# BICLab/Spike2Former

Measured on AMD Instinct MI355X. Metric: fwd+bwd images/sec, 512x512 T=4 ADE20K-150, higher is better.
Workload: dtype f32 (fp32-equivalent: bf16 hi+mid+lo split operands on bf16 MFMA, fp32 accumulate; spike maps stored as bf16, exact); 1 GPU; C2: 512x512 T=4 K=150 Meta-SpikeFormer [64, 128, 256, 360] + MaskFormer head, per-GPU batch 2; global_batch=2, parallelism=dp1, weights=random-init (name-seeded)

## Files before the change

include/s2f.h:

```cpp
#ifndef S2F_H
#define S2F_H

#include <stdint.h>

#ifdef __cplusplus
extern "C" {
#endif

#define S2F_OK 0
#define S2F_EINVAL (-1)
#define S2F_EALIGN (-2)
#define S2F_ELAUNCH (-3)

#define S2F_ABI_VERSION 53
#define S2F_STAT_SLOTS 256

int s2f_version(void);
const char* s2f_last_error(void);

void* s2f_event_create(void);
void s2f_event_destroy(void* event);
int s2f_time_next_call(void* start_event, void* stop_event);
int s2f_event_elapsed_us(void* start_event, void* stop_event, double* microseconds);

int64_t s2f_lif_mask_words(int64_t n);

int s2f_lif_fwd(const float* x, const float* v_in, void* y, float* v_out, uint64_t* mask, uint8_t* count_u8,
                uint64_t* stats, int64_t n, float vth, int D, int y_bf16, void* stream);

int s2f_lif_bwd(const float* gy, const float* gv_out, const uint64_t* mask, float* gx, int64_t n, float vth, int D,
                void* stream);
int s2f_lif_bwd_ports(const float* gy, const float* gy2, const float* gv_out, const uint64_t* mask, const float* skip, float* gx,
                      int64_t n, float vth, int D, void* stream);

int s2f_lif_leaky_fwd(const float* x, const float* v_in, void* y, float* v_out, uint64_t* mask, uint64_t* stats, int64_t n, float vth,
                      int D, float tau, int decay_input, int y_bf16, void* stream);
int s2f_lif_leaky_bwd(const float* gy, const float* gv_out, const uint64_t* mask, float* gx, float* gv_in, int64_t n, float vth, int D,
                      float tau, int decay_input, void* stream);

int s2f_sum2_lif_fwd(const float* x, const float* e, const float* pos, void* y_key, void* y_value, uint64_t* mask_key,
                     uint64_t* mask_value, int64_t TB, int64_t B, int64_t C, int64_t L, float vth, int D, int y_bf16,
                     void* stream);
int s2f_sum2_lif_bwd(const float* g_key, const float* g_value, const uint64_t* mask_key, const uint64_t* mask_value,
                     float* gx, int64_t n, int D, void* stream);
int s2f_sum2_lif_bwd_ex(const float* g_key, const float* g_value, const uint64_t* mask_key, const uint64_t* mask_value, float* gx,
                        float* gx_key, int64_t n, int D, void* stream);
int s2f_sum2_lif_bwd_ports(const float* g_key, const float* g_key2, const float* g_value, const float* g_value2,
                           const uint64_t* mask_key, const uint64_t* mask_value, const float* skip, float* gx, float* gx_key, int64_t n,
                           int D, void* stream);

int s2f_scale_affine_fwd(const float* gamma, const float* beta, const float* s, float* w, float* b, int C, void* stream);
int s2f_scale_affine_bwd(const float* gw, const float* gb, const float* gamma, const float* beta, const float* s,
                         float* dgamma, float* dbeta, float* ds, int C, void* stream);

int s2f_lif_seq_fwd(const float* x_seq, const float* v0, float* y_seq, float* vT, uint64_t* mask, uint64_t* stats,
                    int T, int64_t n, float vth, int D, void* stream);
int s2f_lif_seq_bwd(const float* gy_seq, const float* gvT, const uint64_t* mask, float* gx_seq, float* gv0, int T,
                    int64_t n, float vth, int D, void* stream);

int s2f_bn_single_pass(int64_t N, int64_t C, int64_t L);
int64_t s2f_bn_mask_words(int64_t N, int64_t C, int64_t L);
int s2f_bn_stats(const float* z, const float* conv_bias, double* sums_zeroed, int64_t N, int64_t C, int64_t L,
                 void* stream);
int s2f_bn_act_fwd(const float* z, const float* conv_bias, const double* sums, float* stat_out, float* running_mean,
                   float* running_var, int64_t* num_batches_tracked, const float* gamma, const float* beta,
                   const float* residual, float* u_out, const float* v_in, void* y, float* v_out, uint64_t* mask,
                   uint64_t* stats, int64_t N, int64_t C, int64_t L, float momentum, float eps, int training, float vth,
                   int D, int y_bf16, void* stream);
int s2f_bn_act_bwd(const float* z, const float* conv_bias, const float* stat, const float* gamma, const float* g_u,
                   const float* g_y, const float* g_v, const uint64_t* mask, double* sums_zeroed, float* gz,
                   float* g_residual, float* dgamma, float* dbeta, int64_t N, int64_t C, int64_t L, int training,
                   float vth, int D, void* stream);
int s2f_bn_up_ok(int64_t N, int64_t C, int64_t H, int64_t W, int training, int D);
int s2f_bn_act_up_fwd(const float* z, const float* conv_bias, const double* sums, float* stat_out, float* running_mean,
                      float* running_var, int64_t* num_batches_tracked, const float* gamma, const float* beta,
                      const float* residual_lo, float* u_out, const float* v_in, void* y, float* v_out, uint64_t* mask,
                      uint64_t* stats, int64_t N, int64_t C, int64_t H, int64_t W, float momentum, float eps, int training,
                      float vth, int D, int y_bf16, void* stream);

int s2f_bn2_fused_ok(int64_t N, int64_t C, int64_t L);
int s2f_bn2_act_fwd(const float* z, const float* conv_bias, float* stat_out, float* running_mean, float* running_var,
                    int64_t* num_batches_tracked, const float* gamma, const float* beta, float momentum, float eps,
                    const float* gamma2, const float* beta2, float* running_mean2, float* running_var2,
                    int64_t* num_batches_tracked2, float momentum2, float eps2, const float* residual, float* u_out,
                    const float* v_in, void* y, float* v_out, uint64_t* mask, uint64_t* stats, int64_t N, int64_t C, int64_t L,
                    float vth, int D, int y_bf16, void* stream);
int s2f_bn2_act_bwd(const float* z, const float* conv_bias, const float* stat, const float* gamma, const float* gamma2, float eps2,
                    const float* g_u, const float* g_y, const float* g_v, const uint64_t* mask, float* gz, float* g_residual,
                    float* dgamma, float* dbeta, float* dgamma2, float* dbeta2, int64_t N, int64_t C, int64_t L, float vth, int D,
                    void* stream);

int s2f_im2col(const void* x, void* cols, int N, int C, int H, int W, int kh, int kw, int stride, int pad, int x_bf16, void* stream);
int s2f_col2im(const float* cols, float* gx, int N, int C, int H, int W, int kh, int kw, int stride, int pad, void* stream);
// ... 326 lines not shown
```

spike2former_amd/_lib.py:

```python
import ctypes
import os

import torch

_HERE = os.path.dirname(os.path.abspath(__file__))
LIB_PATH = os.environ.get("S2F_LIB") or os.path.join(_HERE, "libs2f_hip.so")

_p, _i, _i64, _f = ctypes.c_void_p, ctypes.c_int, ctypes.c_int64, ctypes.c_float

SIGNATURES = {
    "s2f_version": (_i, []),
    "s2f_last_error": (ctypes.c_char_p, []),
    "s2f_event_create": (_p, []),
    "s2f_event_destroy": (None, [_p]),
    "s2f_time_next_call": (_i, [_p, _p]),
    "s2f_event_elapsed_us": (_i, [_p, _p, ctypes.POINTER(ctypes.c_double)]),
    "s2f_lif_mask_words": (_i64, [_i64]),
    "s2f_lif_fwd": (_i, [_p, _p, _p, _p, _p, _p, _p, _i64, _f, _i, _i, _p]),
    "s2f_lif_bwd": (_i, [_p, _p, _p, _p, _i64, _f, _i, _p]),
    "s2f_lif_bwd_ports": (_i, [_p] * 6 + [_i64, _f, _i, _p]),
    "s2f_lif_leaky_fwd": (_i, [_p, _p, _p, _p, _p, _p, _i64, _f, _i, _f, _i, _i, _p]),
    "s2f_lif_leaky_bwd": (_i, [_p, _p, _p, _p, _p, _i64, _f, _i, _f, _i, _p]),
    "s2f_sum2_lif_fwd": (_i, [_p] * 7 + [_i64] * 4 + [_f, _i, _i, _p]),
    "s2f_sum2_lif_bwd": (_i, [_p] * 5 + [_i64, _i, _p]),
    "s2f_sum2_lif_bwd_ex": (_i, [_p] * 6 + [_i64, _i, _p]),
    "s2f_sum2_lif_bwd_ports": (_i, [_p] * 9 + [_i64, _i, _p]),
    "s2f_mask_loss_fwd": (_i, [_p] * 4 + [_i64, _i, _i, _f, _f, _p]),
    "s2f_mask_loss_bwd": (_i, [_p] * 5 + [_i64, _i, _i, _f, _f, _p]),
    "s2f_scale_affine_fwd": (_i, [_p] * 5 + [_i, _p]),
    "s2f_scale_affine_bwd": (_i, [_p] * 8 + [_i, _p]),
    "s2f_lif_seq_fwd": (_i, [_p, _p, _p, _p, _p, _p, _i, _i64, _f, _i, _p]),
    "s2f_lif_seq_bwd": (_i, [_p, _p, _p, _p, _p, _i, _i64, _f, _i, _p]),
    "s2f_bn_single_pass": (_i, [_i64] * 3),
    "s2f_bn_mask_words": (_i64, [_i64] * 3),
    "s2f_bn2_fused_ok": (_i, [_i64] * 3),
    "s2f_bn2_act_fwd": (_i, [_p] * 8 + [_f, _f] + [_p] * 5 + [_f, _f] + [_p] * 7 + [_i64] * 3 + [_f, _i, _i, _p]),
    "s2f_bn2_act_bwd": (_i, [_p] * 5 + [_f] + [_p] * 10 + [_i64] * 3 + [_f, _i, _p]),
    "s2f_bn_stats": (_i, [_p] * 3 + [_i64] * 3 + [_p]),
    "s2f_bn_act_fwd": (_i, [_p] * 16 + [_i64] * 3 + [_f, _f, _i, _f, _i, _i, _p]),
    "s2f_bn_act_bwd": (_i, [_p] * 13 + [_i64] * 3 + [_i, _f, _i, _p]),
    "s2f_bn_up_ok": (_i, [_i64] * 4 + [_i, _i]),
    "s2f_bn_act_up_fwd": (_i, [_p] * 16 + [_i64] * 4 + [_f, _f, _i, _f, _i, _i, _p]),
    "s2f_im2col": (_i, [_p, _p] + [_i] * 9 + [_p]),
    "s2f_col2im": (_i, [_p, _p] + [_i] * 8 + [_p]),
    "s2f_dwconv_fwd": (_i, [_p] * 4 + [_i] * 7 + [_p]),
    "s2f_dwconv_stats_slots": (_i64, [_i] * 3),
    "s2f_dwconv_fwd_stats": (_i, [_p] * 4 + [_i64] + [_i] * 5 + [_p]),
    "s2f_dwconv_bn_lif_fwd": (_i, [_p] * 7 + [_f] + [_p] * 3 + [_i] * 7 + [_f, _i, _p]),
    "s2f_dwconv_bwd_input": (_i, [_p] * 3 + [_i] * 6 + [_p]),
    "s2f_dwconv_bwd_weight": (_i, [_p] * 4 + [_i] * 8 + [_p]),
    "s2f_split_bf16x3": (_i, [_p, _p, _i, _i, _i, _i, _p]),
    "s2f_split_bf16x3_multi": (_i, [_p, _i, _i64, _p]),
    "s2f_spike_gemm_fwd": (_i, [_p] * 4 + [_i] * 7 + [_p]),
    "s2f_upsample2x_fwd": (_i, [_p, _p, _i64, _i, _i, _p]),
    "s2f_upsample2x_sigmoid_fwd": (_i, [_p, _p, _i64, _i, _i, _p]),
    "s2f_upsample2x_bwd": (_i, [_p, _p, _i64, _i, _i, _p]),
    "s2f_upsample2x_bwd_add": (_i, [_p, _p, _p, _i64, _i, _i, _p]),
    "s2f_resize_fwd": (_i, [_p, _p, _i64, _i64] + [_i] * 8 + [_p]),
    "s2f_resize_bwd_add": (_i, [_p, _p, _p, _i64] + [_i] * 5 + [_p]),
    "s2f_seg_argmax": (_i, [_p, _p, _p, _i, _i64, _i, _f, _p]),
    "s2f_seg_label": (_i, [_p, _p, _p, _i, _i64] + [_i] * 8 + [_f, _p]),
    "s2f_tta_accumulate": (_i, [_p, _p, _i, _i64] + [_i] * 9 + [_p]),
    "s2f_tta_finish": (_i, [_p, _p, _p, _i, _i64, _i, _f, _p]),
    "s2f_slide_windows": (_i, [_p, _p] + [_i] * 10 + [_p]),
    "s2f_slide_accumulate": (_i, [_p, _p] + [_i] * 10 + [_p]),
    "s2f_seg_hist": (_i, [_p, _i, _p, _i, _i64, _i64, _i, _i64, _i, _i, _i, _p, _p]),
# ... 138 lines not shown
```

spike2former_amd/csrc/bn_lif.hip:

```cpp
#include "gemm_common.h"
#include <cstring>

namespace {

constexpr int kBlock = 256;
constexpr int kWaves = kBlock / S2F_WAVE;

__device__ __forceinline__ double wave_sum_f64(double v) {
  for (int o = 32; o > 0; o >>= 1) v += __shfl_xor(v, o, 64);
  return v;
}

__device__ __forceinline__ void block_atomic_add2(double a, double b, double* dst, double pivot = 0.0, double count = 0.0) {
  __shared__ double red[2 * kWaves];
  a = wave_sum_f64(a);
  b = wave_sum_f64(b);
  const int lane = threadIdx.x & 63, w = threadIdx.x >> 6;
  if (lane == 0) {
    red[2 * w] = a;
    red[2 * w + 1] = b;
  }
  __syncthreads();
  if (threadIdx.x == 0) {
    double sa = 0, sb = 0;
// ... 1067 lines not shown
        }
      }
      if (u_out) st4(u_out + base[i], uo);
      if (LIF) {
        if (YB)
          st4_bf16(y, base[i], yo);
        else
          st4(y + base[i], yo);
        if (v_out) st4(v_out + base[i], vo);
        const uint64_t b0 = __ballot(inr[0]), b1 = __ballot(inr[1]), b2 = __ballot(inr[2]), b3 = __ballot(inr[3]);
        const int64_t tile = base[i] >> 8;
        if (mask != nullptr && lane < 4) mask[tile * 4 + lane] = lane == 0 ? b0 : lane == 1 ? b1 : lane == 2 ? b2 : b3;
      }
    }
  }
  if (LIF && stats != nullptr) {
    double a = (double)csum, bq = (double)cnz;
    block_sum2(a, bq, red, nwaves);
    if (threadIdx.x == 0) {
      unsigned long long* slot = stats + 2 * (blockIdx.x % S2F_STAT_SLOTS);
      if (a > 0) atomicAdd(&slot[0], (unsigned long long)a);
      if (bq > 0) atomicAdd(&slot[1], (unsigned long long)bq);
    }
  }
}

struct Bn2Bwd {
  const float* gamma;
  float* dgamma;
  float* dbeta;
  float eps;
};

template <bool GU, bool GY, bool GV, bool DOUBLE = false>
__global__ __launch_bounds__(kFusedBlock) void bn_fused_bwd_kernel(
    const float* __restrict__ z, const float* __restrict__ bias, const float* __restrict__ stat,
    const float* __restrict__ gamma, const float* __restrict__ g_u, const float* __restrict__ g_y,
    const float* __restrict__ g_v, const uint64_t* __restrict__ mask, float* __restrict__ gz, float* __restrict__ g_res,
    float* __restrict__ dgamma, float* __restrict__ dbeta, int N, int C, int L, double inv_count, float vth, float Df,
    unsigned short* __restrict__ gzs, Bn2Bwd bn2, const float* __restrict__ g_y2) {
  __shared__ double red[2 * kFusedWaves];
  const int c = blockIdx.x, lane = threadIdx.x & 63, w = threadIdx.x >> 6, nwaves = blockDim.x >> 6;
  const int tpr = L >> 8, tiles = N * tpr;
  const float b = bias ? bias[c] : 0.f, mean = stat[c], rstd = stat[C + c], g = gamma[c];
  Tile4 xh[kTpw], gu[kTpw];
  int tix[kTpw];
#pragma unroll
  for (int i = 0; i < kTpw; ++i) {
    const int t = w + i * nwaves;
    tix[i] = t < tiles ? t : -1;
    const int tt = t < tiles ? t : 0;
    const int n = tt / tpr, q = tt - n * tpr;
    const int64_t base = ((int64_t)n * C + c) * L + q * 256 + lane * 4;
    xh[i] = (S2F_BN_NT & 16) ? ld4_nt(z + base) : ld4(z + base);
    if (GU) gu[i] = (S2F_BN_NT & 16) ? ld4_nt(g_u + base) : ld4(g_u + base);
    Tile4 bb, cc;
    uint64_t word = 0;
    if (GY) bb = (S2F_BN_NT & 16) ? ld4_nt(g_y + base) : ld4(g_y + base);
    if (GY && g_y2) {
      const Tile4 t2 = (S2F_BN_NT & 16) ? ld4_nt(g_y2 + base) : ld4(g_y2 + base);
#pragma unroll
      for (int j = 0; j < 4; ++j) bb.a[j] += t2.a[j];
    }
    if (GV) cc = ld4(g_v + base);
    if (GY || GV) word = mask[(base >> 8) * 4 + (lane & 3)];
#pragma unroll
    for (int j = 0; j < 4; ++j) {
      bool m = false;
      if (GY || GV) {
        const uint32_t lo = __shfl((uint32_t)word, j, 64), hi = __shfl((uint32_t)(word >> 32), j, 64);
        m = ((lane < 32 ? lo >> lane : hi >> (lane - 32)) & 1u) != 0;
      }
      gu[i].a[j] = form_gu(GU, GU ? gu[i].a[j] : 0.f, GY, GY ? bb.a[j] : 0.f, GV, GV ? cc.a[j] : 0.f, m, vth, Df);
      xh[i].a[j] = ((xh[i].a[j] + b) - mean) * rstd;
    }
  }
  float ps = 0.f, pq = 0.f;
#pragma unroll
  for (int i = 0; i < kTpw; ++i) {
    if (tix[i] < 0) continue;
#pragma unroll
    for (int j = 0; j < 4; ++j) {
      ps += gu[i].a[j];
      pq += gu[i].a[j] * xh[i].a[j];
    }
  }
  double s1 = (double)ps, s2 = (double)pq;
  block_sum2(s1, s2, red, nwaves);
  float scale = g * rstd;
  float m1 = (float)(s1 * inv_count), m2 = (float)(s2 * inv_count);
  if constexpr (DOUBLE) {
    const float r_c = stat[3 * C + c], g_c = bn2.gamma[c];
    if (threadIdx.x == 0) {
      bn2.dbeta[c] = (float)s1;
      bn2.dgamma[c] = (g * r_c) * (float)s2;
      dbeta[c] = 0.f;
      dgamma[c] = (g_c * bn2.eps) * (r_c * r_c * r_c) * (float)s2;
    }
    scale = (g * rstd) * (g_c * r_c);
    m2 *= (r_c * r_c) * (g * g + bn2.eps);
  } else if (threadIdx.x == 0) {
    dbeta[c] = (float)s1;
    dgamma[c] = (float)s2;
  }
#pragma unroll
  for (int i = 0; i < kTpw; ++i) {
    if (tix[i] < 0) continue;
    const int n = tix[i] / tpr, q = tix[i] - n * tpr;
    const int64_t base = ((int64_t)n * C + c) * L + q * 256 + lane * 4;
    Tile4 o;
#pragma unroll
    for (int j = 0; j < 4; ++j) o.a[j] = scale * ((gu[i].a[j] - m1) - xh[i].a[j] * m2);
    store_gz(gz, gzs, (int64_t)N * C * L, base, o);
    if (g_res) st4(g_res + base, gu[i]);
  }
}

constexpr int kSmallIters = 8;

inline bool small_rows_ok(int64_t N, int64_t C, int64_t L) {
  return (L & 3) == 0 && (L & 255) != 0 && N * L <= 64 * 4 * kSmallIters && N * L >= 8 && C >= 32;
}

template <bool LIF, bool HAS_V, bool YB, bool GROUPED = false>
__global__ __launch_bounds__(64) void bn_small_fwd_kernel(
    const float* __restrict__ z, const float* __restrict__ bias, float* __restrict__ stat, float* __restrict__ running_mean,
    float* __restrict__ running_var, long long* __restrict__ num_batches, const float* __restrict__ gamma,
    const float* __restrict__ beta, const float* __restrict__ res, float* __restrict__ u_out, const float* __restrict__ v_in,
    float* __restrict__ y, float* __restrict__ v_out, uint64_t* __restrict__ mask, unsigned long long* __restrict__ stats,
    int N, int C, int L, double inv_count, float unbias, float momentum, float eps, float vth, float Df) {
  if constexpr (GROUPED) {
    static_assert(!HAS_V, "grouped form: neurons from rest");
    const int64_t g = blockIdx.y, map = g * N * C * L, vec = g * C;
    z += map;
    if (bias) bias += vec;
    stat += 3 * vec;
    if (running_mean) running_mean += vec, running_var += vec;
    gamma += vec, beta += vec;
    if (u_out) u_out += map;
// ... 339 lines not shown
  const float m1 = (float)(s1 * inv_count), m2 = (float)(s2 * inv_count);
#pragma unroll
  for (int i = 0; i < kMidIters; ++i) {
    if (!ok[i]) continue;
    Tile4 o;
#pragma unroll
    for (int j = 0; j < 4; ++j) o.a[j] = (g_ * rstd) * ((gu[i].a[j] - m1) - xh[i].a[j] * m2);
    st4(gz + base[i], o);
    if (g_res) st4(g_res + base[i], gu[i]);
  }
}

inline bool single_pass_ok(int64_t N, int64_t C, int64_t L) {
  if ((L & 255) != 0) return false;
  const int64_t tiles = N * (L >> 8);
  return tiles >= 4 && tiles <= kFusedWaves * kTpw && C >= 64 && N * C * L < ((int64_t)1 << 31);
}
inline int single_pass_threads(int64_t N, int64_t L) {
  const int tiles = (int)(N * (L >> 8));
  return 64 * ((tiles + kTpw - 1) / kTpw);
}

inline int pick_slices(int C, int L, int& slice) {
  int S = 1;
  while ((int64_t)C * S < 1024 && L / (S * 2) >= 2048) S *= 2;
  slice = ((L + S - 1) / S + 3) / 4 * 4;
  return S;
}

inline bool rows_ok(int64_t N, int64_t C, int64_t L, int D) {
  return (L & 3) == 0 && L >= 256 && N * C * L < ((int64_t)1 << 39) && N * C < ((int64_t)1 << 31) && D >= 1 && (D & (D - 1)) == 0;
}
inline bool rows_aligned(int64_t total, int64_t L) { return (L & 255) == 0 && (total & 255) == 0; }
inline bool up_ok(int64_t N, int64_t C, int64_t L, int64_t H, int64_t W, int training, int D) {
  return training && rows_ok(N, C, L, D) && rows_aligned(N * C * L, L) && !single_pass_ok(N, C, L) && H > 0 && W > 0 && H * W == L &&
         (H & 1) == 0 && (W & 3) == 0 && (W < 256 ? 256 % W == 0 : W % 256 == 0) && W < (1 << 24);
}
inline int pick_slices_rows(int C, int L, int& slice) {
  int S = 1;
  while ((int64_t)C * S < 2048 && L / (S * 2) >= 2048) S *= 2;
  slice = ((L + S - 1) / S + 255) / 256 * 256;
  return (L + slice - 1) / slice;
}
template <auto Kern>
int resident_blocks(size_t lds) {
  static int cus = 0, per_cu_small = 0;
  if (cus == 0) {
    int dev = 0;
    if (hipGetDevice(&dev) != hipSuccess || hipDeviceGetAttribute(&cus, hipDeviceAttributeMultiprocessorCount, dev) != hipSuccess ||
        cus < 1)
      cus = 256;
  }
  int per_cu = lds <= 16384 ? per_cu_small : 0;
  if (per_cu == 0) {
    if (hipOccupancyMaxActiveBlocksPerMultiprocessor(&per_cu, Kern, kBlock, lds <= 16384 ? 16384 : lds) != hipSuccess || per_cu < 1)
      per_cu = 4;
    if (lds <= 16384) per_cu_small = per_cu;
  }
  return cus * per_cu;
}
template <auto Kern>
int grid_rows(uint32_t ntiles, size_t lds, uint32_t& chunk, int want) {
  static const char* env = getenv("S2F_BN_ROWS_CHUNK");
  if (env != nullptr) {
    const int fwd_want = atoi(env), bwd_want = strchr(env, ',') ? atoi(strchr(env, ',') + 1) : fwd_want;
    want = want == 8 ? fwd_want : bwd_want;
// ... 32 lines not shown
    {true, true, true},
};
template <class F>
void for_fwd_variant(const float* y, const float* v_in, int y_bf16, const F& launch) {
  s2f_dispatch<kFwdVariants>(
      [&](const FwdVariant& e) {
        return y ? (e.lif && e.has_v == (v_in != nullptr) && e.yb == (y_bf16 != 0)) : !e.lif;
      },
      launch);
}

struct BwdGrads {
  bool gu, gy, gv;
};
constexpr BwdGrads kBwdGrads[] = {
    {false, false, true},
    {false, true, false},
    {false, true, true},
    {true, false, false},
    {true, false, true},
    {true, true, false},
    {true, true, true},
};
template <class F>
void for_bwd_grads(const float* g_u, const float* g_y, const float* g_v, const F& launch) {
  s2f_dispatch<kBwdGrads>(
      [&](const BwdGrads& e) { return e.gu == (g_u != nullptr) && e.gy == (g_y != nullptr) && e.gv == (g_v != nullptr); }, launch);
}

}

extern "C" int s2f_bn_single_pass(int64_t N, int64_t C, int64_t L) {
  return (single_pass_ok(N, C, L) || small_rows_ok(N, C, L) || mid_rows_ok(N, C, L)) ? 1 : 0;
}

extern "C" int64_t s2f_bn_mask_words(int64_t N, int64_t C, int64_t L) {
  if (small_rows_ok(N, C, L)) return C * kSmallIters * 4;
  if (mid_rows_ok(N, C, L)) return C * kMidIters * kMidWaves * 4;
  return ((N * C * L + 255) >> 8) * 4;
}

extern "C" int s2f_bn_stats(const float* z, const float* conv_bias, double* sums_zeroed, int64_t N, int64_t C, int64_t L,
                            void* stream) {
  S2F_REQUIRE(z && sums_zeroed, S2F_EINVAL, "s2f_bn_stats: null z/workspace");
  int rc = check_shape("s2f_bn_stats", N, C, L);
  if (rc) return rc;
  int slice;
  const int S = pick_slices((int)C, (int)L, slice);
  if (L & 3) {
    S2F_LAUNCH(true, true, bn_stats_any_kernel, dim3((unsigned)C, S), dim3(kBlock), 0, (hipStream_t)stream, z, conv_bias,
               sums_zeroed, (int)N, (int)C, (int)L, slice);
    return s2f_check_launch("s2f_bn_stats");
  }
  S2F_REQUIRE(s2f_aligned16(z), S2F_EALIGN, "s2f_bn_stats: z must be 16-byte aligned");
  S2F_LAUNCH(true, true, bn_stats_kernel, dim3((unsigned)C, S), dim3(kBlock), 0, (hipStream_t)stream, z, conv_bias,
                     sums_zeroed, (int)N, (int)C, (int)L, slice);
  return s2f_check_launch("s2f_bn_stats");
}

extern "C" int s2f_bn_partials_finalize(const float* partials, int64_t P, const float* conv_bias, double* sums_out, int64_t N,
                                        int64_t C, int64_t L, void* stream) {
  S2F_REQUIRE(partials && sums_out && P > 0 && P < (1 << 24) && (reinterpret_cast<uintptr_t>(partials) & 7u) == 0, S2F_EINVAL,
              "s2f_bn_partials_finalize: partials 8-byte aligned, 0 < P < 2^24, sums workspace given");
  int rc = check_shape("s2f_bn_partials_finalize", N, C, L);
  if (rc) return rc;
  const int per_wave = P <= 256;
// ... 116 lines not shown
                                 float* v_out, uint64_t* mask, uint64_t* stats, int64_t N, int64_t C, int64_t H, int64_t W,
                                 float momentum, float eps, int training, float vth, int D, int y_bf16, void* stream) {
  S2F_REQUIRE(H > 0 && W > 0 && (H & 1) == 0 && (W & 1) == 0, S2F_EINVAL, "s2f_bn_act_up_fwd: even H, W");
  return bn_act_fwd_impl(z, conv_bias, sums, stat_out, running_mean, running_var, num_batches_tracked, gamma, beta, residual_lo,
                         u_out, v_in, y_out, v_out, mask, stats, N, C, H * W, momentum, eps, training, vth, D, y_bf16, stream, Bn2{},
                         H / 2, W / 2);
}

extern "C" int s2f_bn2_fused_ok(int64_t N, int64_t C, int64_t L) { return single_pass_ok(N, C, L) ? 1 : 0; }

extern "C" int s2f_bn2_act_fwd(const float* z, const float* conv_bias, float* stat_out, float* running_mean, float* running_var,
                               int64_t* num_batches_tracked, const float* gamma, const float* beta, float momentum, float eps,
                               const float* gamma2, const float* beta2, float* running_mean2, float* running_var2,
                               int64_t* num_batches_tracked2, float momentum2, float eps2, const float* residual, float* u_out,
                               const float* v_in, void* y_out, float* v_out, uint64_t* mask, uint64_t* stats, int64_t N, int64_t C,
                               int64_t L, float vth, int D, int y_bf16, void* stream) {
  S2F_REQUIRE(gamma2 && beta2, S2F_EINVAL, "s2f_bn2_act_fwd: null second BatchNorm");
  return bn_act_fwd_impl(z, conv_bias, nullptr, stat_out, running_mean, running_var, num_batches_tracked, gamma, beta, residual, u_out,
                         v_in, y_out, v_out, mask, stats, N, C, L, momentum, eps, 1, vth, D, y_bf16, stream,
                         Bn2{gamma2, beta2, running_mean2, running_var2, reinterpret_cast<long long*>(num_batches_tracked2), eps2,
                             momentum2});
}

static int bn_act_bwd_impl(const float* z, const float* conv_bias, const float* stat, const float* gamma, const float* g_u,
                           const float* g_y, const float* g_v, const uint64_t* mask, double* sums_zeroed, float* gz,
                           float* g_residual, float* dgamma, float* dbeta, int64_t N, int64_t C, int64_t L, int training,
                           float vth, int D, void* stream, unsigned short* gzs, Bn2Bwd bn2 = Bn2Bwd{}, const float* g_y2 = nullptr) {
  S2F_REQUIRE(!g_y2 || (g_y && s2f_aligned16(g_y2) && !(training && (mid_rows_ok(N, C, L) || small_rows_ok(N, C, L))) &&
                        ((training && single_pass_ok(N, C, L)) || rows_ok(N, C, L, D))),
              S2F_EINVAL, "s2f_bn_act_bwd_ports: a second spike gradient only on the single-pass and row-walking kernels (s2f_bn_bwd_ports_ok)");
  S2F_REQUIRE(!bn2.gamma || (training && single_pass_ok(N, C, L) && bn2.dgamma && bn2.dbeta && !gzs), S2F_EINVAL,
              "s2f_bn2_act_bwd: the BatchNorm pair runs on the single-pass kernels only");
  const bool single = training && (single_pass_ok(N, C, L) || small_rows_ok(N, C, L) || mid_rows_ok(N, C, L));
  S2F_REQUIRE(z && stat && gamma && (single || sums_zeroed) && (gz || gzs) && dgamma && dbeta, S2F_EINVAL,
              "s2f_bn_act_bwd: null pointer");
  S2F_REQUIRE(!gzs || (reinterpret_cast<uintptr_t>(gzs) & 7u) == 0, S2F_EALIGN, "s2f_bn_act_bwd_split: gz_split must be 8-byte aligned");
  S2F_REQUIRE(g_u || g_y || g_v, S2F_EINVAL, "s2f_bn_act_bwd: no incoming gradient");
  S2F_REQUIRE(!(g_y || g_v) || mask, S2F_EINVAL, "s2f_bn_act_bwd: spike gradients need the in-range mask");
  int rc = check_shape("s2f_bn_act_bwd", N, C, L);
  if (rc) return rc;
  hipStream_t s = (hipStream_t)stream;
  const int64_t total = N * C * L;
  const double inv_count = 1.0 / ((double)N * (double)L);
  if (training && mid_rows_ok(N, C, L)) {
    S2F_REQUIRE(gzs == nullptr && gz, S2F_EINVAL, "s2f_bn_act_bwd_split: rows that are not whole tiles have no bf16-plane form");
    for_bwd_grads(g_u, g_y, g_v, [&](auto i) {
      constexpr BwdGrads G = kBwdGrads[i];
      S2F_LAUNCH(true, true, (bn_mid_bwd_kernel<G.gu, G.gy, G.gv>), dim3((unsigned)C), dim3(mid_rows_threads(N, L)), 0, s, z,
                 conv_bias, stat, gamma, g_u, g_y, g_v, mask, gz, g_residual, dgamma, dbeta, (int)N, (int)C, (int)L, inv_count,
                 vth, (float)D);
    });
    return s2f_check_launch("s2f_bn_act_bwd");
  }
  if (training && small_rows_ok(N, C, L)) {
    S2F_REQUIRE(gzs == nullptr && gz, S2F_EINVAL, "s2f_bn_act_bwd_split: short rows (N * L <= 2048) have no bf16-plane form");
    for_bwd_grads(g_u, g_y, g_v, [&](auto i) {
      constexpr BwdGrads G = kBwdGrads[i];
      S2F_LAUNCH(true, true, (bn_small_bwd_kernel<G.gu, G.gy, G.gv>), dim3((unsigned)C), dim3(64), 0, s, z, conv_bias, stat,
                 gamma, g_u, g_y, g_v, mask, gz, g_residual, dgamma, dbeta, (int)N, (int)C, (int)L, inv_count, vth, (float)D);
    });
    return s2f_check_launch("s2f_bn_act_bwd");
  }
  if (single) {
    for_bwd_grads(g_u, g_y, g_v, [&](auto i) {
      constexpr BwdGrads G = kBwdGrads[i];
      s2f_dispatch_bool(bn2.gamma != nullptr, [&](auto pair) {
        S2F_LAUNCH(true, true, (bn_fused_bwd_kernel<G.gu, G.gy, G.gv, pair.value>), dim3((unsigned)C),
                   dim3(single_pass_threads(N, L)), 0, s, z, conv_bias, stat, gamma, g_u, g_y, g_v, mask, gz, g_residual, dgamma,
                   dbeta, (int)N, (int)C, (int)L, inv_count, vth, (float)D, gzs, bn2, g_y2);
      });
    });
    return s2f_check_launch("s2f_bn_act_bwd");
  }
  if (rows_ok(N, C, L, D)) {
    int slice;
    const int S = pick_slices_rows((int)C, (int)L, slice);
    const uint32_t ntiles = (uint32_t)((total + 255) >> 8);
    for_bwd_grads(g_u, g_y, g_v, [&](auto i) {
      constexpr BwdGrads G = kBwdGrads[i];
      S2F_LAUNCH(true, false, (bn_bwd_reduce_rows_kernel<G.gu, G.gy, G.gv>), dim3((unsigned)C, S), dim3(kBlock), 0, s, z,
                 conv_bias, stat, g_u, g_y, g_v, mask, sums_zeroed, (int)N, (int)C, (int)L, slice, vth, (float)D, g_y2);
      s2f_dispatch_bool(rows_aligned(total, L), [&](auto al) {
        uint32_t chunk;
        const int rgrid = grid_rows<bn_bwd_apply_rows_kernel<G.gu, G.gy, G.gv, al.value>>(ntiles, 0, chunk, 4);
        S2F_LAUNCH(false, true, (bn_bwd_apply_rows_kernel<G.gu, G.gy, G.gv, al.value>), dim3(rgrid), dim3(kBlock), 0, s, z,
                   conv_bias, stat, gamma, g_u, g_y, g_v, mask, sums_zeroed, gz, g_residual, dgamma, dbeta, total, ntiles,
                   (int)C, (uint32_t)L, chunk, inv_count, training, vth, (float)D, gzs, g_y2);
      });
    });
    return s2f_check_launch("s2f_bn_act_bwd");
  }
  int slice;
  const int S = pick_slices((int)C, (int)L, slice);
  const bool anyl = (L & 3) != 0;
  S2F_REQUIRE(!anyl || gzs == nullptr, S2F_EINVAL, "s2f_bn_act_bwd_split: rows of L %% 4 != 0 elements have no bf16-plane form");
  S2F_LAUNCH(true, false, anyl ? bn_bwd_reduce_any_kernel : bn_bwd_reduce_kernel, dim3((unsigned)C, S), dim3(kBlock), 0, s, z,
             conv_bias, stat, g_u, g_y, g_v, mask, sums_zeroed, (int)N, (int)C, (int)L, slice, vth, (float)D);
  s2f_dispatch_bool(anyl, [&](auto al) {
    S2F_LAUNCH(false, true, bn_bwd_apply_kernel<al.value>, dim3(grid_flat(total)), dim3(kBlock), 2 * C * sizeof(float), s, z,
               conv_bias, stat, gamma, g_u, g_y, g_v, mask, sums_zeroed, gz, g_residual, dgamma, dbeta, total, (int)C, (int)L,
               inv_count, training, vth, (float)D, gzs);
  });
// ... 101 lines not shown
```

spike2former_amd/ops/bn.py:

```python
import torch

from .config import cfg
from .core import *
from .resize import upsample_bilinear


class _BNAct(torch.autograd.Function):

    @staticmethod
    def forward(ctx, z, conv_bias, gamma, beta, residual, v_in, running_mean, running_var, nbt, training, momentum,
                eps, lif_on, want_pre, keep_v, D, vth, stats, bf16, partials=None, up_lo=None, up_skip=False, groups=1):
        _need_cuda(z, conv_bias, gamma, beta, residual, v_in, up_lo)
        ctx.groups = groups
        if groups > 1:
            return _BNAct._forward_siblings(ctx, z, conv_bias, gamma, beta, running_mean, running_var, momentum, eps, lif_on, want_pre,
                                            D, vth, bf16, groups, plain=(residual is None and v_in is None and nbt is None and training
                                                                         and not keep_v and stats is None and up_lo is None))
        up_in = up_lo
        z = z.contiguous()
        N, C = z.shape[0], z.shape[1]
        L = z.numel() // (N * C)
        dev = z.device
        stat = torch.empty(3 * C, dtype=torch.float32, device=dev)
        s = _stream()
# ... 94 lines not shown

    @staticmethod
    def backward(ctx, g_u, g_y, g_v, g_border, _g_ydata, g_y2, g_through=None):
        z, conv_bias, gamma, stat, mask = ctx.saved_tensors
        N, C, L, training, D, vth, has_res, has_bias = ctx.cfg

        def prep(g):
            return None if (g is None or g.numel() == 0) else g.contiguous()
        g_u, g_y, g_v, g_y2 = prep(g_u), prep(g_y), prep(g_v), prep(g_y2)
        if ctx.groups > 1:
            if g_u is None and g_y is None:
                return (None,) * 23
            G = ctx.groups
            gz = torch.empty_like(z)
            dgamma = torch.empty(G * C, dtype=torch.float32, device=z.device)
            dbeta = torch.empty(G * C, dtype=torch.float32, device=z.device)
            alg = 4 * z.numel() * (2 + (g_u is not None) + (g_y is not None))
            _time_next("bn_lif_bwd" if g_y is not None else "bn_bwd", alg)
            check(lib.s2f_bn_act_bwd_grouped(_ptr(z), _ptr(conv_bias), _ptr(stat), _ptr(gamma), _ptr(g_u), _ptr(g_y), _ptr(mask),
                                             _ptr(gz), _ptr(dgamma), _ptr(dbeta), G, N, C, L, vth, D, _stream()),
                  "s2f_bn_act_bwd_grouped")
            return (gz, None, dgamma, dbeta) + (None,) * 19
        if g_y is None:
            g_y, g_y2 = g_y2, None
        if g_y2 is not None and not lib.s2f_bn_bwd_ports_ok(N, C, L, int(training), D):
            g_y, g_y2 = g_y + g_y2, None
        if g_u is None and g_y is None and g_v is None:
            return (None,) * 20 + (g_through, None, None)
        dev = z.device
        gz = torch.empty_like(z)
        g_res = torch.empty_like(z) if ((has_res and ctx.needs_input_grad[4]) or (ctx.up is not None and ctx.needs_input_grad[20])) else None
        dgamma = torch.empty(C, dtype=torch.float32, device=dev)
        dbeta = torch.empty(C, dtype=torch.float32, device=dev)
        ws = None if (training and lib.s2f_bn_single_pass(N, C, L)) else _take_zeroed(2 * C, dev)
        alg = 4 * z.numel() * (2 + (g_u is not None) + (g_y is not None) + (g_res is not None))
        _time_next("bn_lif_bwd" if g_y is not None else "bn_bwd", alg, moved=alg + 4 * z.numel() * (g_y2 is not None))
        check(lib.s2f_bn_act_bwd_ports(_ptr(z), _ptr(conv_bias), _ptr(stat), _ptr(gamma), _ptr(g_u), _ptr(g_y), _ptr(g_y2), _ptr(g_v),
                                       _ptr(mask), _ptr(ws), _ptr(gz), _ptr(g_res), _ptr(dgamma), _ptr(dbeta), N, C, L,
                                       int(training), vth, D, _stream()), "s2f_bn_act_bwd_ports")
        g_bias = None
        if has_bias:
            g_bias = None if training else gamma * stat[C:2 * C] * dbeta
        if ctx.needs_input_grad[5]:
            raise RuntimeError("gradient w.r.t. the incoming membrane is not supported by the fused BN+LIF op")
        if ctx.up is not None:
            g_lo = g_through
            if g_res is not None:
                h, w = ctx.up
                g_lo = torch.empty(N, C, h, w, dtype=torch.float32, device=dev)
                check(lib.s2f_upsample2x_bwd_add(_ptr(g_res), _ptr(None if g_through is None else g_through.contiguous()), _ptr(g_lo),
                                                 N * C, h, w, _stream()), "s2f_upsample2x_bwd_add")
            return (gz, g_bias, dgamma, dbeta, None) + (None,) * 15 + (g_lo, None, None)
        return (gz, g_bias, dgamma, dbeta, g_res) + (None,) * 18


def _partial_slots(z):
    N, C = z.shape[0], z.shape[1]
    out = (int(lib.s2f_bn_partials_count(N, z.numel() // (N * C))),)
    if z.dim() == 4:
        out += (int(lib.s2f_dwconv_stats_slots(N, z.shape[2], z.shape[3])),)
    return out


def bn_up_ok(z, lo, training, D=8):
    if not (training and z.dim() == 4 and lo.dim() == 4 and z.is_cuda and lo.is_cuda and z.dtype == lo.dtype == torch.float32
            and z.numel() and lo.shape[:2] == z.shape[:2] and (2 * lo.shape[2], 2 * lo.shape[3]) == tuple(z.shape[2:])):
        return False
# ... 158 lines not shown
```

spike2former_amd/ops/config.py:

```python
import os


class Config:
    FIELDS = ("KERNEL_EVENTS", "GRAD_SINKS", "WGRAD_STREAM", "BRANCH_STREAMS", "LONG_STREAMS", "LONG_WHAT", "SPIKES_BF16",
              "SPIKE_GEMM_TERMS", "SPIKE_GEMM_ENABLED", "SPIKE_GEMM_CHECK", "CONV3X3_IMPLICIT", "CONV3X3_IMPLICIT_MIN_PIXELS",
              "CONV3X3_DX_IMPLICIT", "DEFER_DW", "DW_PIPE", "BN_PARTIALS", "BN_PARTIALS_SINGLE", "DENSE_GROUPED", "RESPLIT_IN_GRAPH",
              "FANOUT_PORTS", "GLUE_MODE", "STRICT_GLUE", "STRICT", "GENERAL_RESIZE")
    RUNTIME = ("KERNEL_EVENTS", "GRAD_SINKS", "WGRAD_STREAM", "BRANCH_STREAMS", "LONG_STREAMS")
    LAUNCH_FIELDS = ("DECODER_SIBLINGS", "DCN_CHANNEL_MAJOR")

    def __setattr__(self, name, value):
        if name not in self.FIELDS and name not in self.LAUNCH_FIELDS:
            raise AttributeError(f"ops.cfg has no switch {name!r} (the switches are ops.cfg.FIELDS)")
        object.__setattr__(self, name, value)

    def __init__(self):
        self.KERNEL_EVENTS = None
        self.GRAD_SINKS = None
        self.WGRAD_STREAM = None
        self.DEFER_DW = True
        self.BRANCH_STREAMS = None
        self.LONG_STREAMS = None
        self.LONG_WHAT = ("lat", "mf", "kv")
        self.SPIKES_BF16 = True
        self.SPIKE_GEMM_TERMS = 3
        self.SPIKE_GEMM_ENABLED = True
        self.CONV3X3_IMPLICIT = True
        self.CONV3X3_IMPLICIT_MIN_PIXELS = int(os.environ.get("S2F_CONV3_MIN_PIXELS", 32 * 32))
        self.CONV3X3_DX_IMPLICIT = True
        self.DW_PIPE = os.environ.get("S2F_DW_PIPE", "1") != "0"
        self.SPIKE_GEMM_CHECK = False
        self.BN_PARTIALS = os.environ.get("S2F_BN_PARTIALS", "1") != "0"
        self.BN_PARTIALS_SINGLE = os.environ.get("S2F_BN_PARTIALS_SINGLE", "0") != "0"
        self.DENSE_GROUPED = os.environ.get("S2F_DENSE_GROUPED", "1") != "0"
        self.RESPLIT_IN_GRAPH = True
        self.FANOUT_PORTS = os.environ.get("S2F_FANOUT_PORTS", "1") != "0"
        self.GLUE_MODE = os.environ.get("S2F_GLUE_MODE", "0") != "0"
        self.STRICT_GLUE = os.environ.get("S2F_STRICT_GLUE", "0") != "0"
        self.STRICT = os.environ.get("S2F_STRICT", "0") != "0"
        self.GENERAL_RESIZE = True
        self.DECODER_SIBLINGS = os.environ.get("S2F_DEC_SIBLINGS", "1") != "0"
        self.DCN_CHANNEL_MAJOR = os.environ.get("S2F_DCN_CM", "1") != "0"

    def snapshot(self):
        return {n: getattr(self, n) for n in self.FIELDS if n not in self.RUNTIME and n not in ("STRICT", "STRICT_GLUE")}

    def launch_snapshot(self):
        return dict(self.snapshot(), **{n: getattr(self, n) for n in self.LAUNCH_FIELDS})


cfg = Config()
```

Before: 57.32 images/s.

## Add wide one-pass fused BN+LIF backward for mid-sized channel rows

Adds a wider template variant of the fused BatchNorm+LIF backward kernel that holds up to eight tiles per wave in registers. Rows too large for the existing single-pass path but small enough for this width now run in one kernel per channel instead of the separate stats-reduction and apply passes with a zeroed double workspace. Mask words are loaded once per lane and spread with readlane and inverse ballot, and the extra gradient loads are grouped with scheduling barriers to limit register pressure. The cost is higher VGPR use and lower occupancy, and it only applies where N*L/256 tiles fall within the new window and C>=64.

Result: no change. 57.53 images/s (median of 6 runs) (+0.4%).

```diff
diff --git a/include/s2f.h b/include/s2f.h
--- a/include/s2f.h
+++ b/include/s2f.h
@@ -12,7 +12,7 @@
 #define S2F_EALIGN (-2)
 #define S2F_ELAUNCH (-3)
 
-#define S2F_ABI_VERSION 53
+#define S2F_ABI_VERSION 54
 #define S2F_STAT_SLOTS 256
 
 int s2f_version(void);
@@ -59,6 +59,7 @@
                     int64_t n, float vth, int D, void* stream);
 
 int s2f_bn_single_pass(int64_t N, int64_t C, int64_t L);
+int s2f_bn_bwd_one_pass(int64_t N, int64_t C, int64_t L, int D);
 int64_t s2f_bn_mask_words(int64_t N, int64_t C, int64_t L);
 int s2f_bn_stats(const float* z, const float* conv_bias, double* sums_zeroed, int64_t N, int64_t C, int64_t L,
                  void* stream);
diff --git a/spike2former_amd/_lib.py b/spike2former_amd/_lib.py
--- a/spike2former_amd/_lib.py
+++ b/spike2former_amd/_lib.py
@@ -32,6 +32,7 @@
     "s2f_lif_seq_fwd": (_i, [_p, _p, _p, _p, _p, _p, _i, _i64, _f, _i, _p]),
     "s2f_lif_seq_bwd": (_i, [_p, _p, _p, _p, _p, _i, _i64, _f, _i, _p]),
     "s2f_bn_single_pass": (_i, [_i64] * 3),
+    "s2f_bn_bwd_one_pass": (_i, [_i64] * 3 + [_i]),
     "s2f_bn_mask_words": (_i64, [_i64] * 3),
     "s2f_bn2_fused_ok": (_i, [_i64] * 3),
     "s2f_bn2_act_fwd": (_i, [_p] * 8 + [_f, _f] + [_p] * 5 + [_f, _f] + [_p] * 7 + [_i64] * 3 + [_f, _i, _i, _p]),
diff --git a/spike2former_amd/csrc/bn_lif.hip b/spike2former_amd/csrc/bn_lif.hip
--- a/spike2former_amd/csrc/bn_lif.hip
+++ b/spike2former_amd/csrc/bn_lif.hip
@@ -1123,7 +1123,9 @@
   float eps;
 };
 
-template <bool GU, bool GY, bool GV, bool DOUBLE = false>
+constexpr int kTpwWide = 8;
+
+template <bool GU, bool GY, bool GV, bool DOUBLE = false, int TPW = kTpw, bool GY2 = false>
 __global__ __launch_bounds__(kFusedBlock) void bn_fused_bwd_kernel(
     const float* __restrict__ z, const float* __restrict__ bias, const float* __restrict__ stat,
     const float* __restrict__ gamma, const float* __restrict__ g_u, const float* __restrict__ g_y,
@@ -1131,13 +1133,79 @@
     float* __restrict__ dgamma, float* __restrict__ dbeta, int N, int C, int L, double inv_count, float vth, float Df,
     unsigned short* __restrict__ gzs, Bn2Bwd bn2, const float* __restrict__ g_y2) {
   __shared__ double red[2 * kFusedWaves];
-  const int c = blockIdx.x, lane = threadIdx.x & 63, w = threadIdx.x >> 6, nwaves = blockDim.x >> 6;
+  constexpr bool WIDE = TPW > kTpw;
+  static_assert(!(WIDE && DOUBLE), "the BatchNorm pair is tied to the single-pass forward: at most kFusedWaves * kTpw tiles");
+  static_assert(!GY2 || (WIDE && GY), "GY2: the wide form with a spike gradient");
+  const int c = blockIdx.x, lane = threadIdx.x & 63, nwaves = blockDim.x >> 6;
+  const int w = WIDE ? __builtin_amdgcn_readfirstlane((int)(threadIdx.x >> 6)) : (int)(threadIdx.x >> 6);
   const int tpr = L >> 8, tiles = N * tpr;
   const float b = bias ? bias[c] : 0.f, mean = stat[c], rstd = stat[C + c], g = gamma[c];
-  Tile4 xh[kTpw], gu[kTpw];
-  int tix[kTpw];
-#pragma unroll
-  for (int i = 0; i < kTpw; ++i) {
+  Tile4 xh[TPW], gu[TPW];
+  int tix[TPW];
+  if constexpr (WIDE) {
+    constexpr int kExtra = (GU && GY ? 1 : 0) + (GY2 ? 1 : 0) + ((GU || GY) && GV ? 1 : 0);
+    constexpr int kGroup = kExtra <= 1 ? 4 : kExtra == 2 ? 2 : 1;
+    auto base_of = [&](int i) __attribute__((always_inline)) {
+      const int tt = tix[i] < 0 ? 0 : tix[i];
+      const int n = tt / tpr, q = tt - n * tpr;
+      return ((int64_t)n * C + c) * L + q * 256;
+    };
+    uint32_t l4 = (uint32_t)lane * 4u;
+    uint64_t mw = 0;
+    if (GY || GV) {
+      const int t = w + (lane >> 2) * nwaves, tt = (lane >> 2) < TPW && t < tiles ? t : w;
+      const int n = tt / tpr, q = tt - n * tpr;
+      mw = mask[(((int64_t)n * C + c) * tpr + q) * 4 + (lane & 3)];
+    }
+#pragma unroll
+    for (int i = 0; i < TPW; ++i) {
+      const int t = w + i * nwaves;
+      tix[i] = t < tiles ? t : -1;
+      const int64_t base = base_of(i);
+      xh[i] = (S2F_BN_NT & 16) ? ld4_nt(z + base + l4) : ld4(z + base + l4);
+      const float* first = (GU ? g_u : GY ? g_y : g_v) + base;
+      gu[i] = (S2F_BN_NT & 16) && (GU || GY) ? ld4_nt(first + l4) : ld4(first + l4);
+    }
+#pragma unroll
+    for (int i0 = 0; i0 < TPW; i0 += kGroup) {
+      Tile4 bb[kGroup], cc[kGroup];
+#pragma unroll
+      for (int k = 0; k < kGroup; ++k) {
+        const int64_t base = base_of(i0 + k);
+        if (GY) bb[k] = GU ? ((S2F_BN_NT & 16) ? ld4_nt(g_y + base + l4) : ld4(g_y + base + l4)) : gu[i0 + k];
+        if (GV) cc[k] = (GU || GY) ? ld4(g_v + base + l4) : gu[i0 + k];
+      }
+      if (GY2) {
+#pragma unroll
+        for (int k = 0; k < kGroup; ++k) {
+          const int64_t base = base_of(i0 + k);
+          const Tile4 t2 = (S2F_BN_NT & 16) ? ld4_nt(g_y2 + base + l4) : ld4(g_y2 + base + l4);
+#pragma unroll
+          for (int j = 0; j < 4; ++j) bb[k].a[j] += t2.a[j];
+        }
+      }
+#pragma unroll
+      for (int k = 0; k < kGroup; ++k) {
+        const int i = i0 + k;
+#pragma unroll
+        for (int j = 0; j < 4; ++j) {
+          bool m = false;
+          if (GY || GV) {
+            const uint32_t lo = __builtin_amdgcn_readlane((uint32_t)mw, 4 * i + j), hi = __builtin_amdgcn_readlane((uint32_t)(mw >> 32), 4 * i + j);
+            m = __builtin_amdgcn_inverse_ballot_w64(((uint64_t)hi << 32) | lo);
+          }
+          gu[i].a[j] = form_gu(GU, GU ? gu[i].a[j] : 0.f, GY, GY ? bb[k].a[j] : 0.f, GV, GV ? cc[k].a[j] : 0.f, m, vth, Df);
+          xh[i].a[j] = ((xh[i].a[j] + b) - mean) * rstd;
+        }
+      }
+      if (kExtra > 0) {
+        asm volatile("" : "+v"(l4) : "v"(gu[i0].a[0]), "v"(gu[i0 + kGroup - 1].a[3]));
+        __builtin_amdgcn_sched_barrier(0);
+      }
+    }
+  }
+#pragma unroll
+  for (int i = 0; i < (WIDE ? 0 : TPW); ++i) {
     const int t = w + i * nwaves;
     tix[i] = t < tiles ? t : -1;
     const int tt = t < tiles ? t : 0;
@@ -1168,7 +1236,7 @@
   }
   float ps = 0.f, pq = 0.f;
 #pragma unroll
-  for (int i = 0; i < kTpw; ++i) {
+  for (int i = 0; i < TPW; ++i) {
     if (tix[i] < 0) continue;
 #pragma unroll
     for (int j = 0; j < 4; ++j) {
@@ -1195,7 +1263,7 @@
     dgamma[c] = (float)s2;
   }
 #pragma unroll
-  for (int i = 0; i < kTpw; ++i) {
+  for (int i = 0; i < TPW; ++i) {
     if (tix[i] < 0) continue;
     const int n = tix[i] / tpr, q = tix[i] - n * tpr;
     const int64_t base = ((int64_t)n * C + c) * L + q * 256 + lane * 4;
@@ -1601,6 +1669,16 @@
   return (L & 3) == 0 && L >= 256 && N * C * L < ((int64_t)1 << 39) && N * C < ((int64_t)1 << 31) && D >= 1 && (D & (D - 1)) == 0;
 }
 inline bool rows_aligned(int64_t total, int64_t L) { return (L & 255) == 0 && (total & 255) == 0; }
+constexpr int kOnePassMinC = 64;
+inline bool bwd_one_pass_ok(int64_t N, int64_t C, int64_t L, int D) {
+  if ((L & 255) != 0 || !rows_ok(N, C, L, D)) return false;
+  const int64_t tiles = N * (L >> 8);
+  return tiles > kFusedWaves * kTpw && tiles <= kFusedWaves * kTpwWide && C >= kOnePassMinC && N * C * L < ((int64_t)1 << 31);
+}
+inline int bwd_one_pass_threads(int64_t N, int64_t L) {
+  const int tiles = (int)(N * (L >> 8));
+  return 64 * ((tiles + kTpwWide - 1) / kTpwWide);
+}
 inline bool up_ok(int64_t N, int64_t C, int64_t L, int64_t H, int64_t W, int training, int D) {
   return training && rows_ok(N, C, L, D) && rows_aligned(N * C * L, L) && !single_pass_ok(N, C, L) && H > 0 && W > 0 && H * W == L &&
          (H & 1) == 0 && (W & 3) == 0 && (W < 256 ? 256 % W == 0 : W % 256 == 0) && W < (1 << 24);
@@ -1699,6 +1777,11 @@
 
 extern "C" int s2f_bn_single_pass(int64_t N, int64_t C, int64_t L) {
   return (single_pass_ok(N, C, L) || small_rows_ok(N, C, L) || mid_rows_ok(N, C, L)) ? 1 : 0;
+}
+
+extern "C" int s2f_bn_bwd_one_pass(int64_t N, int64_t C, int64_t L, int D) {
+  if (N <= 0 || C <= 0 || L <= 0) return 0;
+  return (bwd_one_pass_ok(N, C, L, D) && !single_pass_ok(N, C, L) && !small_rows_ok(N, C, L) && !mid_rows_ok(N, C, L)) ? 1 : 0;
 }
 
 extern "C" int64_t s2f_bn_mask_words(int64_t N, int64_t C, int64_t L) {
@@ -1881,8 +1964,9 @@
   S2F_REQUIRE(!bn2.gamma || (training && single_pass_ok(N, C, L) && bn2.dgamma && bn2.dbeta && !gzs), S2F_EINVAL,
               "s2f_bn2_act_bwd: the BatchNorm pair runs on the single-pass kernels only");
   const bool single = training && (single_pass_ok(N, C, L) || small_rows_ok(N, C, L) || mid_rows_ok(N, C, L));
-  S2F_REQUIRE(z && stat && gamma && (single || sums_zeroed) && (gz || gzs) && dgamma && dbeta, S2F_EINVAL,
-              "s2f_bn_act_bwd: null pointer");
+  const bool wide = training && !single && sums_zeroed == nullptr && !bn2.gamma && bwd_one_pass_ok(N, C, L, D);
+  S2F_REQUIRE(z && stat && gamma && (single || wide || sums_zeroed) && (gz || gzs) && dgamma && dbeta, S2F_EINVAL,
+              "s2f_bn_act_bwd: null pointer (the sums workspace may be left out only where s2f_bn_single_pass or s2f_bn_bwd_one_pass)");
   S2F_REQUIRE(!gzs || (reinterpret_cast<uintptr_t>(gzs) & 7u) == 0, S2F_EALIGN, "s2f_bn_act_bwd_split: gz_split must be 8-byte aligned");
   S2F_REQUIRE(g_u || g_y || g_v, S2F_EINVAL, "s2f_bn_act_bwd: no incoming gradient");
   S2F_REQUIRE(!(g_y || g_v) || mask, S2F_EINVAL, "s2f_bn_act_bwd: spike gradients need the in-range mask");
@@ -1917,6 +2001,18 @@
         S2F_LAUNCH(true, true, (bn_fused_bwd_kernel<G.gu, G.gy, G.gv, pair.value>), dim3((unsigned)C),
                    dim3(single_pass_threads(N, L)), 0, s, z, conv_bias, stat, gamma, g_u, g_y, g_v, mask, gz, g_residual, dgamma,
                    dbeta, (int)N, (int)C, (int)L, inv_count, vth, (float)D, gzs, bn2, g_y2);
+      });
+    });
+    return s2f_check_launch("s2f_bn_act_bwd");
+  }
+  if (wide) {
+    for_bwd_grads(g_u, g_y, g_v, [&](auto i) {
+      constexpr BwdGrads G = kBwdGrads[i];
+      s2f_dispatch_bool(g_y2 != nullptr, [&](auto y2) {
+        if constexpr (G.gy || !y2.value)
+          S2F_LAUNCH(true, true, (bn_fused_bwd_kernel<G.gu, G.gy, G.gv, false, kTpwWide, y2.value>), dim3((unsigned)C),
+                     dim3(bwd_one_pass_threads(N, L)), 0, s, z, conv_bias, stat, gamma, g_u, g_y, g_v, mask, gz, g_residual, dgamma,
+                     dbeta, (int)N, (int)C, (int)L, inv_count, vth, (float)D, gzs, Bn2Bwd{}, g_y2);
       });
     });
     return s2f_check_launch("s2f_bn_act_bwd");
diff --git a/spike2former_amd/ops/bn.py b/spike2former_amd/ops/bn.py
--- a/spike2former_amd/ops/bn.py
+++ b/spike2former_amd/ops/bn.py
@@ -150,7 +150,8 @@
         g_res = torch.empty_like(z) if ((has_res and ctx.needs_input_grad[4]) or (ctx.up is not None and ctx.needs_input_grad[20])) else None
         dgamma = torch.empty(C, dtype=torch.float32, device=dev)
         dbeta = torch.empty(C, dtype=torch.float32, device=dev)
-        ws = None if (training and lib.s2f_bn_single_pass(N, C, L)) else _take_zeroed(2 * C, dev)
+        one_pass = training and (lib.s2f_bn_single_pass(N, C, L) or (cfg.BN_BWD_ONE_PASS and lib.s2f_bn_bwd_one_pass(N, C, L, D)))
+        ws = None if one_pass else _take_zeroed(2 * C, dev)
         alg = 4 * z.numel() * (2 + (g_u is not None) + (g_y is not None) + (g_res is not None))
         _time_next("bn_lif_bwd" if g_y is not None else "bn_bwd", alg, moved=alg + 4 * z.numel() * (g_y2 is not None))
         check(lib.s2f_bn_act_bwd_ports(_ptr(z), _ptr(conv_bias), _ptr(stat), _ptr(gamma), _ptr(g_u), _ptr(g_y), _ptr(g_y2), _ptr(g_v),
diff --git a/spike2former_amd/ops/config.py b/spike2former_amd/ops/config.py
--- a/spike2former_amd/ops/config.py
+++ b/spike2former_amd/ops/config.py
@@ -7,7 +7,7 @@
               "CONV3X3_DX_IMPLICIT", "DEFER_DW", "DW_PIPE", "BN_PARTIALS", "BN_PARTIALS_SINGLE", "DENSE_GROUPED", "RESPLIT_IN_GRAPH",
               "FANOUT_PORTS", "GLUE_MODE", "STRICT_GLUE", "STRICT", "GENERAL_RESIZE")
     RUNTIME = ("KERNEL_EVENTS", "GRAD_SINKS", "WGRAD_STREAM", "BRANCH_STREAMS", "LONG_STREAMS")
-    LAUNCH_FIELDS = ("DECODER_SIBLINGS", "DCN_CHANNEL_MAJOR")
+    LAUNCH_FIELDS = ("DECODER_SIBLINGS", "DCN_CHANNEL_MAJOR", "BN_BWD_ONE_PASS")
 
     def __setattr__(self, name, value):
         if name not in self.FIELDS and name not in self.LAUNCH_FIELDS:
@@ -41,6 +41,7 @@
         self.GENERAL_RESIZE = True
         self.DECODER_SIBLINGS = os.environ.get("S2F_DEC_SIBLINGS", "1") != "0"
         self.DCN_CHANNEL_MAJOR = os.environ.get("S2F_DCN_CM", "1") != "0"
+        self.BN_BWD_ONE_PASS = os.environ.get("S2F_BN_BWD_ONE_PASS", "1") != "0"
 
     def snapshot(self):
         return {n: getattr(self, n) for n in self.FIELDS if n not in self.RUNTIME and n not in ("STRICT", "STRICT_GLUE")}
```
